# josegarciav/PINNs-RL-PDE

Hardware: AMD Instinct MI355X
Metric: collocation-points/sec (residual+grad) + final residual L2, Burgers 1D (higher is better)
Workload: dtype f32

## Files before the change

### pinns-rl-pde_amd/csrc/jet_kernel_u16.h

```cpp
#pragma once
#include "jet_kernel_wide.h"

namespace pinn {

#define U16_BARRIER(idx)     \
  do {                       \
    PINN_STAMP(idx);         \
    __syncthreads();         \
    PINN_STAMP(ST_BARRIER);  \
  } while (0)

constexpr int kU = 16;
constexpr int kUP = 132;
constexpr int kUThreads = 512;
constexpr int kUWaves = 8;
constexpr int kUH = 128;
constexpr int kUImgS = kU * kUP;

__device__ __forceinline__ f32x4 mfma16(float a, float b, f32x4 c) {
  return __builtin_amdgcn_mfma_f32_16x16x4f32(a, b, c, 0, 0, 0);
}

__device__ __forceinline__ int u16_opaque(int v) {
  asm volatile("" : "+v"(v));
// ... 87 lines not shown
__device__ __forceinline__ void u16_gemm_n(f32x4 (&acc)[K], const float* W, int ld, unsigned off, f32x4 w0, f32x4 w1, const float* xl) {
  f32x4 wq[3];
  wq[0] = w0;
  wq[1] = w1;
  f32x4 bc[K], bn[K];
#pragma unroll
  for (int s = 0; s < K; ++s) bc[s] = *reinterpret_cast<const f32x4*>(xl + s * kUImgS);
#pragma unroll
  for (int b = 0; b < NB; ++b) {
    if (b + 2 < NB) wq[(b + 2) % 3] = u16_wload<COLS>(W, ld, off, b + 2);
    if (b + 1 < NB) {
#pragma unroll
      for (int s = 0; s < K; ++s) bn[s] = *reinterpret_cast<const f32x4*>(xl + s * kUImgS + 16 * (b + 1));
    }
    __builtin_amdgcn_sched_barrier(0);
#pragma unroll
    for (int m = 0; m < 4; ++m)
#pragma unroll
      for (int s = 0; s < K; ++s) acc[s] = mfma16(wq[b % 3][m], bc[s][m], acc[s]);
    __builtin_amdgcn_sched_barrier(0);
    if (b + 1 < NB) {
#pragma unroll
      for (int s = 0; s < K; ++s) bc[s] = bn[s];
    }
  }
}

template <int K, bool COLS>
__device__ __forceinline__ void u16_gemm(f32x4 (&acc)[K], const float* W, int ld, unsigned off, f32x4 w0, f32x4 w1, int nb, const float* xl) {
  switch (nb) {
    case 8: u16_gemm_n<K, 8, COLS>(acc, W, ld, off, w0, w1, xl); return;
    case 4: u16_gemm_n<K, 4, COLS>(acc, W, ld, off, w0, w1, xl); return;
    default: break;
  }
#pragma unroll 1
  for (int b = 0; b < nb; ++b) {
    const f32x4 w = b == 0 ? w0 : b == 1 ? w1 : u16_wload<COLS>(W, ld, off, b);
#pragma unroll
    for (int m = 0; m < 4; ++m)
#pragma unroll
      for (int s = 0; s < K; ++s) acc[s] = mfma16(w[m], xl[s * kUImgS + 16 * b + m], acc[s]);
  }
}

template <int K, int NA, int OFF, int NPT>
__device__ __forceinline__ void u16_outer_n(f32x4 (&pt)[NPT], const float* zl, const float* al) {
  float zc, zn, ac[NA], an[NA];
  zc = zl[0];
#pragma unroll
  for (int t = 0; t < NA; ++t) ac[t] = al[16 * t];
#pragma unroll
  for (int st = 0; st < 4 * K; ++st) {
    if (st + 1 < 4 * K) {
      const int s = (st + 1) >> 2, m = (st + 1) & 3;
      zn = zl[s * kUImgS + m * kUP];
#pragma unroll
      for (int t = 0; t < NA; ++t) an[t] = al[s * kUImgS + m * kUP + 16 * t];
    }
    __builtin_amdgcn_sched_barrier(0);
#pragma unroll
    for (int t = 0; t < NA; ++t) pt[OFF + t] = mfma16(zc, ac[t], pt[OFF + t]);
    __builtin_amdgcn_sched_barrier(0);
    if (st + 1 < 4 * K) {
      zc = zn;
#pragma unroll
      for (int t = 0; t < NA; ++t) ac[t] = an[t];
    }
  }
}

template <int K, int OFF, int NMAX, int NPT>
__device__ __forceinline__ void u16_outer(f32x4 (&pt)[NPT], int na, const float* zl, const float* al) {
  if constexpr (NMAX >= 8) {
    if (na * 2 == NMAX) { u16_outer_n<K, NMAX / 2, OFF, NPT>(pt, zl, al); return; }
  }
  u16_outer_n<K, NMAX, OFF, NPT>(pt, zl, al);
}

#ifndef PINN_U16_PACK
#define PINN_U16_PACK 1
#endif
constexpr int kUPackMax = 3;

template <int NB, bool COLS>
__device__ __forceinline__ void u16p_gemm_n(f32x4 (&acc)[kUPackMax], int G, const float* W, int ld, unsigned off, f32x4 w0, f32x4 w1, const float* xl) {
  f32x4 wq[3];
  wq[0] = w0;
  wq[1] = w1;
  f32x4 bc[kUPackMax], bn[kUPackMax];
#pragma unroll
  for (int j = 0; j < kUPackMax; ++j) {
    bc[j] = f32x4{0.0f, 0.0f, 0.0f, 0.0f};
    bn[j] = bc[j];
    if (j < G) bc[j] = *reinterpret_cast<const f32x4*>(xl + 4 * j * kUP);
  }
#pragma unroll
  for (int b = 0; b < NB; ++b) {
    if (b + 2 < NB) wq[(b + 2) % 3] = u16_wload<COLS>(W, ld, off, b + 2);
    if (b + 1 < NB) {
#pragma unroll
      for (int j = 0; j < kUPackMax; ++j)
        if (j < G) bn[j] = *reinterpret_cast<const f32x4*>(xl + 4 * j * kUP + 16 * (b + 1));
    }
#pragma unroll
    for (int j = 0; j < kUPackMax; ++j) {
      if (j < G) {
#pragma unroll
        for (int m = 0; m < 4; ++m) acc[j] = mfma16(wq[b % 3][m], bc[j][m], acc[j]);
      }
    }
    if (b + 1 < NB) {
#pragma unroll
      for (int j = 0; j < kUPackMax; ++j) bc[j] = bn[j];
    }
  }
}

template <bool COLS>
__device__ __forceinline__ void u16p_gemm(f32x4 (&acc)[kUPackMax], int G, const float* W, int ld, unsigned off, f32x4 w0, f32x4 w1, int nb, const float* xl) {
  switch (nb) {
    case 8: u16p_gemm_n<8, COLS>(acc, G, W, ld, off, w0, w1, xl); return;
    case 4: u16p_gemm_n<4, COLS>(acc, G, W, ld, off, w0, w1, xl); return;
    default: break;
  }
#pragma unroll 1
  for (int b = 0; b < nb; ++b) {
    const f32x4 w = b == 0 ? w0 : b == 1 ? w1 : u16_wload<COLS>(W, ld, off, b);
#pragma unroll
    for (int j = 0; j < kUPackMax; ++j) {
      if (j < G) {
#pragma unroll
        for (int m = 0; m < 4; ++m) acc[j] = mfma16(w[m], xl[4 * j * kUP + 16 * b + m], acc[j]);
      }
    }
  }
}

template <int K, int NA, int OFF, int NPT>
__device__ __forceinline__ void u16p_outer_n(f32x4 (&pt)[NPT], int G, const float* zl, const float* al) {
#pragma unroll
  for (int j = 0; j < kUPackMax; ++j) {
    if (j < G) {
      float zc, zn = 0.0f, ac[NA], an[NA];
      zc = zl[4 * j * kUP];
#pragma unroll
      for (int t = 0; t < NA; ++t) {
        ac[t] = al[4 * j * kUP + 16 * t];
        an[t] = 0.0f;
      }
#pragma unroll
      for (int s = 0; s < K; ++s) {
        if (s + 1 < K) {
          zn = zl[(s + 1) * kUImgS + 4 * j * kUP];
#pragma unroll
          for (int t = 0; t < NA; ++t) an[t] = al[(s + 1) * kUImgS + 4 * j * kUP + 16 * t];
        }
        __builtin_amdgcn_sched_barrier(0);
#pragma unroll
        for (int t = 0; t < NA; ++t) pt[OFF + t] = mfma16(zc, ac[t], pt[OFF + t]);
        __builtin_amdgcn_sched_barrier(0);
        if (s + 1 < K) {
          zc = zn;
#pragma unroll
          for (int t = 0; t < NA; ++t) ac[t] = an[t];
        }
      }
// ... 9 lines not shown
  u16p_outer_n<K, NMAX, OFF, NPT>(pt, G, zl, al);
}

__device__ __forceinline__ void u16_wave_sync() {
  __builtin_amdgcn_fence(__ATOMIC_RELEASE, "wavefront");
  __builtin_amdgcn_wave_barrier();
  __builtin_amdgcn_fence(__ATOMIC_ACQUIRE, "wavefront");
}

template <int ACT, int NT, int NX, bool MRG = false>
__device__ __forceinline__ void u16_ew_forward(f32x4 (&v)[1 + NT + NX], float w, f32x4 (&rec)[1 + NT + NX], float cc = 0.0f) {
  constexpr int K = 1 + NT + NX;
#pragma unroll
  for (int r = 0; r < 4; ++r) {
    float z[K], y[K];
#pragma unroll
    for (int s = 0; s < K; ++s) z[s] = v[s][r];
    if constexpr (MRG) act_fwd_merged<ACT>(w, cc, z, y);
    else act_fwd<ACT, NT, NX>(w, z, y);
    rec[0][r] = ActTape<ACT>::value_is_output ? y[0] : z[0];
#pragma unroll
    for (int s = 1; s < K; ++s) rec[s][r] = z[s];
#pragma unroll
    for (int s = 0; s < K; ++s) v[s][r] = y[s];
  }
}

template <int K>
__device__ __forceinline__ void u16_put(float* il, const f32x4 (&v)[K]) {
#pragma unroll
  for (int s = 0; s < K; ++s) *reinterpret_cast<f32x4*>(il + s * kUImgS) = v[s];
}
template <int K>
__device__ __forceinline__ void u16_get(const float* il, f32x4 (&v)[K]) {
#pragma unroll
  for (int s = 0; s < K; ++s) v[s] = *reinterpret_cast<const f32x4*>(il + s * kUImgS);
}

template <int ACT, int NT, int NX, bool MRG = false>
__device__ __forceinline__ float u16_ew_backward(f32x4 (&ab)[1 + NT + NX], float w, const f32x4 (&rec)[1 + NT + NX], float cc = 0.0f) {
  constexpr int K = 1 + NT + NX;
  float part = 0.0f;
#pragma unroll
  for (int r = 0; r < 4; ++r) {
    float z[K], abv[K], zb[K];
#pragma unroll
    for (int s = 0; s < K; ++s) {
      z[s] = rec[s][r];
      abv[s] = ab[s][r];
    }
    if constexpr (MRG) part += act_bwd_tape_merged<ACT>(w, cc, z, abv, zb);
    else act_bwd_tape<ACT, NT, NX>(w, z, abv, zb);
#pragma unroll
    for (int s = 0; s < K; ++s) ab[s][r] = zb[s];
  }
  return part;
}

template <int ACT, int NT, int NX, bool MRG>
__device__ __forceinline__ void u16_act_replay(float w, float cc, const float* z, float* y) {
  if constexpr (MRG) act_fwd_tape_merged<ACT>(w, cc, z, y);
  else act_fwd_tape<ACT, NT, NX>(w, z, y);
}

__device__ __forceinline__ f32x4 row16_sum4(f32x4 v) {
#pragma unroll
  for (int r = 0; r < 4; ++r) v[r] = row16_sum(v[r]);
  return v;
}

template <int ACT, int NT, int NX, bool BWD, int NA0, bool COEF = false, bool MRG = false>
__global__ __launch_bounds__(kUThreads, 1) void jet_kernel_u16(const KernelArgs a) {
  static_assert(!MRG || (NT == 1 && NX == 1), "the merged set is laid out as the (1,1) set");
  constexpr int K = 1 + NT + NX;
  constexpr int NKT = kUH / 16;
  constexpr int NPT = NA0 + (kPersist - 1) * NKT;
  static_assert(kPersist == 3, "the layer -> tile-offset table below is written for three persistent layers");
  constexpr int img = K * kUImgS;
  extern __shared__ __attribute__((aligned(16))) float smem[];
  const NetDev& net = a.net;
  float* X = smem;
  float* A2 = X + img;
  float* REC = A2 + img;
  float* UP = REC + 2 * img;
  float* xin2 = UP + kUWaves * K * kU;
  float* wb = xin2 + 2 * kMaxDin * kU;
  float* ep = wb + (1 + kPersist) * kUH;
  float* pl = ep + (kMaxDin + 1) * kUH;
  float* pdwl = pl + (kPersist + kMaxDin + 1) * kUH;
  float* psl = pdwl + 4 * kUThreads;
  float* xint = psl + 2 * kU;
  [[maybe_unused]] float* pcl = xint + kMaxDin * kU;
  auto mcoef = [&]() -> float {
    if constexpr (MRG) return -X[kUH + 2];
    else return 0.0f;
  };
  auto cadd = [&](float part, bool own) {
    if constexpr (MRG && COEF) {
      if (own) pcl[u16_opaque(threadIdx.x)] += part;
    }
  };

  PINN_STAMP_DECL
  const int tid = threadIdx.x;
  const int wv = __builtin_amdgcn_readfirstlane(tid >> 6);
  const int lane = tid & 63;
  const int g = lane >> 4, c = lane & 15;
  const int din = net.din;
  const int nl = net.n_layers;
#if PINN_U16_PACK
  const long long NL = a.u16_loop_points;
#else
  const long long NL = a.N;
#endif
  const long long nunits = (NL + kU - 1) / kU;
  const int frow = 16 * wv + 4 * g;
  const int ioff = c * kUP + frow;

  for (int k = tid; k < kUH; k += kUThreads) {
    wb[k] = k < net.h_last ? net.w_out[k] : 0.0f;
    for (int l = 0; l < nl; ++l) wb[(1 + l) * kUH + k] = k < net.layer[l].out_dim ? net.layer[l].b[k] : 0.0f;
  }
  stage_enc_params<kUH>(net, ep, tid);
#pragma unroll
  for (int i = 0; i < kPersist + kMaxDin + 1; ++i)
    if (tid < kUH) pl[i * kUH + tid] = 0.0f;
  const float b_out0 = net.b_out[0];
  static_assert(!COEF || BWD, "coefficient cotangents belong to the reverse launch");
  if constexpr (COEF) {
    if (tid < kU) {
      X[tid * kUP + kUH] = 0.0f;
      X[tid * kUP + kUH + 1] = 0.0f;
    }
  }
  if (tid < 4) {
    const float cv = tid == 0 ? a.pde.c0 : tid == 1 ? a.pde.c1 : tid == 2 ? a.pde.c2 : a.pde.c3;
    X[tid * kUP + kUH + 2] = COEF ? a.pde.coef_dev[tid] : cv;
  }

  f32x4 pt[NPT];
#pragma unroll
  for (int t = 0; t < NPT; ++t) pt[t] = f32x4{0.0f, 0.0f, 0.0f, 0.0f};
  if constexpr (BWD) *reinterpret_cast<f32x4*>(pdwl + 4 * tid) = f32x4{0.0f, 0.0f, 0.0f, 0.0f};
  if (tid < 2 * kU) psl[tid] = 0.0f;
  if constexpr (MRG && COEF) pcl[tid] = 0.0f;

  float xr[kMaxDin] = {0.0f, 0.0f, 0.0f, 0.0f};
  auto fetch_coords = [&](long long u) {
    if (tid < kU) {
      const long long p = u * kU + tid;
      const bool ok = u < nunits && p < NL;
#pragma unroll
      for (int cc = 0; cc < kMaxDin; ++cc) {
        if (cc < din - 1) xr[cc] = ok ? a.x[p * (din - 1) + cc] : 0.0f;
        if (cc == din - 1) xr[cc] = ok ? a.t[p] : 0.0f;
      }
    }
  };
  auto fetch_coords_at = [&](long long p0, int npts) {
    if (tid < kU) {
      const long long p = p0 + tid;
      const bool ok = tid < npts && p < a.N;
#pragma unroll
      for (int cc = 0; cc < kMaxDin; ++cc) {
        if (cc < din - 1) xr[cc] = ok ? a.x[p * (din - 1) + cc] : 0.0f;
        if (cc == din - 1) xr[cc] = ok ? a.t[p] : 0.0f;
      }
    }
  };
  auto put_coords = [&](float* dst) {
    if (tid < kU) {
#pragma unroll
      for (int cc = 0; cc < kMaxDin; ++cc) dst[cc * kU + tid] = xr[cc];
    }
  };
#if PINN_U16_PACK
  if (a.u16_tail_groups > 0) {
    fetch_coords_at(a.u16_loop_points + 4LL * a.u16_tail_groups * blockIdx.x, 4 * a.u16_tail_groups);
    put_coords(xint);
  }
#endif
  fetch_coords(blockIdx.x);
  put_coords(xin2);
  int xpar = 0;

  for (long long u = blockIdx.x; u < nunits; u += gridDim.x) {
    const long long p0 = u * kU;
    U16_BARRIER(ST_BWD_FLUSH);
    const float* xin = xin2 + xpar * (kMaxDin * kU);
    float* xin_next = xin2 + (xpar ^ 1) * (kMaxDin * kU);
    xpar ^= 1;
    fetch_coords(u + gridDim.x);
    f32x4 w0, w1;
    {
      const LayerDev L0 = uniform_layer(net.layer[0]);
      const unsigned off = u16_rows_off(16 * wv < L0.out_dim ? 16 * wv : 0, L0.ld, c, g);
      w0 = u16_wload<false>(L0.W, L0.ld, off, 0);
      w1 = u16_wload<false>(L0.W, L0.ld, off, L0.in_dim > 16 ? 1 : 0);
    }
    PINN_STAMP(ST_STAGE);
    float* src = (nl & 1) ? X : A2;
    float* dst = (nl & 1) ? A2 : X;
    u16_encode<ACT, NT, NX, MRG>(net, ep, xin, src, u16_opaque(tid), mcoef());
    U16_BARRIER(ST_ENCODE);

    f32x4 acc[K];
    for (int l = 0; l < nl; ++l) {
      const LayerDev Ly = uniform_layer(net.layer[l]);
      const bool on = 16 * wv < Ly.out_dim;
      const bool last = l + 1 == nl;
#pragma unroll
      for (int s = 0; s < K; ++s) acc[s] = f32x4{0.0f, 0.0f, 0.0f, 0.0f};
      if (on) {
        u16_gemm<K, false>(acc, Ly.W, Ly.ld, u16_rows_off(16 * wv, Ly.ld, c, g), w0, w1, Ly.in_dim >> 4, src + c * kUP + 4 * g);
        acc[0] += *reinterpret_cast<const f32x4*>(wb + (1 + l) * kUH + frow);
      }
      if (l == 0) put_coords(xin_next);
      PINN_STAMP(ST_FWD_GEMM);
      if (!last) {
        {
          const LayerDev Ln = uniform_layer(net.layer[l + 1]);
          const unsigned off = u16_rows_off(16 * wv < Ln.out_dim ? 16 * wv : 0, Ln.ld, c, g);
          w0 = u16_wload<false>(Ln.W, Ln.ld, off, 0);
          w1 = u16_wload<false>(Ln.W, Ln.ld, off, Ln.in_dim > 16 ? 1 : 0);
        }
        if (on) {
          f32x4 rec[K];
          u16_ew_forward<ACT, NT, NX, MRG>(acc, Ly.act_param, rec, mcoef());
          if constexpr (BWD) u16_put<K>(REC + l * img + ioff, rec);
        }
        if (on) u16_put<K>(dst + ioff, acc);
        U16_BARRIER(ST_FWD_EW);
        float* const t = src;
        src = dst;
        dst = t;
      } else if (on) {
        f32x4 rec[K];
        u16_ew_forward<ACT, NT, NX, MRG>(acc, Ly.act_param, rec, mcoef());
        if constexpr (BWD) u16_put<K>(A2 + ioff, rec);
      }
    }
    PINN_STAMP(ST_FWD_EW);

    {
      const f32x4 w4 = *reinterpret_cast<const f32x4*>(wb + frow);
      float po[K];
#pragma unroll
      for (int s = 0; s < K; ++s) {
        po[s] = fmaf(w4[0], acc[s][0], fmaf(w4[1], acc[s][1], fmaf(w4[2], acc[s][2], w4[3] * acc[s][3])));
        po[s] += __shfl_xor(po[s], 16);
        po[s] += __shfl_xor(po[s], 32);
      }
      if (g == 0) {
#pragma unroll
        for (int s = 0; s < K; ++s) UP[(wv * K + s) * kU + c] = po[s];
      }
    }
    U16_BARRIER(ST_OUT);

    float ub[K];
    {
      const long long p = p0 + c;
      const bool ok = p < NL;
      const bool writer = tid < kU;
      float j[K];
#pragma unroll
      for (int s = 0; s < K; ++s) {
        float v = s == 0 ? b_out0 : 0.0f;
#pragma unroll
        for (int w = 0; w < kUWaves; ++w) v += UP[(w * K + s) * kU + c];
        j[s] = v;
      }
      if (a.mode == MODE_JETS) {
#pragma unroll
        for (int s = 0; s < K; ++s) {
          if (writer && ok && a.jets_out[s]) a.jets_out[s][p] = j[s];
          ub[s] = (BWD && ok && a.jets_bar[s]) ? a.jets_bar[s][p] : 0.0f;
        }
      } else {
        float d[K];
        PdeDev pde = a.pde;
        pde.c0 = X[0 * kUP + kUH + 2];
        pde.c1 = X[1 * kUP + kUH + 2];
        pde.c2 = X[2 * kUP + kUH + 2];
        pde.c3 = X[3 * kUP + kUH + 2];
        float r;
        if constexpr (MRG) r = pde_residual_merged(j, d);
        else r = pde_residual<NT, NX>(pde, j, xin[c], d);
        float dl;
        float lt = loss_term(pde, r, &dl);
        if (!ok) {
          lt = 0.0f;
          dl = 0.0f;
        }
        if (writer && ok && a.residual_out) a.residual_out[p] = r;
        if (writer) psl[c] += lt;
        const float rb = !BWD ? 0.0f : a.res_bar ? (ok ? a.res_bar[p] : 0.0f) : a.grad_scale * dl;
#pragma unroll
        for (int s = 0; s < K; ++s) ub[s] = rb * d[s];
        if constexpr (COEF && !MRG) {
          float dc0, dc1;
          pde_coef_grads<NT, NX>(pde, j, xin[c], dc0, dc1);
          if (writer) {
            X[c * kUP + kUH] += rb * dc0;
            X[c * kUP + kUH + 1] += rb * dc1;
          }
        }
      }
    }

    PINN_STAMP(ST_EPI);
    if constexpr (!BWD) continue;
    if (tid < kU) psl[kU + c] += ub[0];
    f32x4 ab[K];
    {
      const LayerDev Lz = uniform_layer(net.layer[nl - 1]);
      const f32x4 w4 = *reinterpret_cast<const f32x4*>(wb + frow);
#pragma unroll
      for (int s = 0; s < K; ++s) ab[s] = w4 * ub[s];
      if (16 * wv < Lz.out_dim) {
        f32x4 rec[K];
        u16_get<K>(A2 + ioff, rec);
        float* const pdwp = pdwl + 4 * u16_opaque(tid);
        f32x4 pdw = *reinterpret_cast<const f32x4*>(pdwp);
#pragma unroll
        for (int r = 0; r < 4; ++r) {
          float z[K], y[K];
#pragma unroll
          for (int s = 0; s < K; ++s) z[s] = rec[s][r];
          u16_act_replay<ACT, NT, NX, MRG>(Lz.act_param, mcoef(), z, y);
          float gg = 0.0f;
#pragma unroll
          for (int s = 0; s < K; ++s) gg = fmaf(ub[s], y[s], gg);
          pdw[r] += gg;
        }
        *reinterpret_cast<f32x4*>(pdwp) = pdw;
        cadd(u16_ew_backward<ACT, NT, NX, MRG>(ab, Lz.act_param, rec, mcoef()), true);
      }
    }
    PINN_STAMP(ST_B0);

    for (int l = nl - 1; l >= 0; --l) {
      const LayerDev Ly = uniform_layer(net.layer[l]);
      const bool on = 16 * wv < Ly.out_dim;
      const bool need_abar = l > 0 || net.enc == ENC_LINEAR;
      const bool kon = 16 * wv < Ly.in_dim;
      if (l + 1 < nl || nl == 1) U16_BARRIER(ST_BWD_EW);
      if (on) u16_put<K>(X + ioff, ab);
      float pw = 0.0f;
      if (l > 0) {
        const LayerDev P = uniform_layer(net.layer[l - 1]);
        pw = P.act_param;
        if (kon) {
          f32x4 rec[K], y[K];
          u16_get<K>(REC + (l - 1) * img + ioff, rec);
#pragma unroll
          for (int r = 0; r < 4; ++r) {
            float z[K], yy[K];
#pragma unroll
            for (int s = 0; s < K; ++s) z[s] = rec[s][r];
            u16_act_replay<ACT, NT, NX, MRG>(pw, mcoef(), z, yy);
#pragma unroll
            for (int s = 0; s < K; ++s) y[s][r] = yy[s];
          }
          u16_put<K>(A2 + ioff, y);
        }
      } else {
        u16_encode<ACT, NT, NX, MRG>(net, ep, xin, A2, u16_opaque(tid), mcoef());
      }
      const unsigned coff = u16_cols_off(kon ? 16 * wv : 0, Ly.ld, c, g);
      if (need_abar) {
        w0 = u16_wload<true>(Ly.W, Ly.ld, coff, 0);
        w1 = u16_wload<true>(Ly.W, Ly.ld, coff, 1);
      }
      U16_BARRIER(ST_BWD_PUT);
      if (Ly.db && tid < Ly.out_dim) {
        float gsum = 0.0f;
#pragma unroll
        for (int n = 0; n < kU; ++n) gsum += X[n * kUP + tid];
        pl[l * kUH + tid] += gsum;
      }
      PINN_STAMP(ST_BWD_DB);
      const bool dw_first = wv >= 4;
#pragma unroll
      for (int half = 0; half < 2; ++half) {
        if ((half == 0) == dw_first && on && Ly.dW) {
          const float* zl = X + 4 * g * kUP + 16 * wv + c;
          const float* al = A2 + 4 * g * kUP + c;
          const int na = Ly.in_dim >> 4;
          if (l == 0) u16_outer<K, 0, NA0, NPT>(pt, na, zl, al);
          else if (l == 1) u16_outer<K, NA0, NKT, NPT>(pt, na, zl, al);
          else u16_outer<K, NA0 + NKT, NKT, NPT>(pt, na, zl, al);
        }
        if ((half == 0) == dw_first) PINN_STAMP(ST_BWD_STREAM);
        if (half == 1) break;
        if (need_abar) {
#pragma unroll
          for (int s = 0; s < K; ++s) ab[s] = f32x4{0.0f, 0.0f, 0.0f, 0.0f};
          if (kon) u16_gemm<K, true>(ab, Ly.W, Ly.ld, coff, w0, w1, Ly.out_dim >> 4, X + c * kUP + 4 * g);
        }
        PINN_STAMP(ST_BWD_DX);
        if (l > 0 && kon) {
          f32x4 rec[K];
          u16_get<K>(REC + (l - 1) * img + ioff, rec);
          cadd(u16_ew_backward<ACT, NT, NX, MRG>(ab, pw, rec, mcoef()), true);
        }
        PINN_STAMP(ST_BWD_EW);
      }
      if constexpr (MRG && COEF) {
        if (l == 0 && net.enc == ENC_FOURIER && kon) {
          f32x4 aw[1] = {f32x4{0.0f, 0.0f, 0.0f, 0.0f}};
          {
            const float* xl = X + kUImgS + c * kUP + 4 * g;
            const int nb = Ly.out_dim >> 4;
#pragma unroll 1
            for (int b = 0; b < nb; ++b) {
              const f32x4 w = u16_wload<true>(Ly.W, Ly.ld, coff, b);
              const f32x4 xv = *reinterpret_cast<const f32x4*>(xl + 16 * b);
#pragma unroll
              for (int m = 0; m < 4; ++m) aw[0] = mfma16(w[m], xv[m], aw[0]);
            }
          }
          const int M = net.enc_out >> 1;
          const f32x4 val = *reinterpret_cast<const f32x4*>(A2 + ioff);
          float part = 0.0f;
#pragma unroll
          for (int r = 0; r < 4; ++r) {
            const int jf = frow + r;
            part = fmaf(aw[0][r], fourier_coef_partial_merged(ep[jf < M ? jf : jf - M], val[r]), part);
          }
          cadd(part, true);
        }
      }
    }

    if (net.enc == ENC_LINEAR && (net.d_encW || (MRG && COEF))) {
      const int H = net.enc_out;
      const bool enc_sums = !(MRG && COEF) || net.d_encW != nullptr;
      U16_BARRIER(ST_ENC_BWD);
      if (16 * wv < H) {
#pragma unroll
        for (int r = 0; r < 4; ++r) {
          float z[K], abv[K], zb[K];
          u16_enc_preact<NT, NX>(ep, din, xin, frow + r, c, z);
#pragma unroll
          for (int s = 0; s < K; ++s) abv[s] = ab[s][r];
          if constexpr (MRG) cadd(act_bwd_merged<ACT>(net.enc_param, mcoef(), z, abv, zb), true);
          else act_bwd<ACT, NT, NX>(net.enc_param, z, abv, zb);
#pragma unroll
          for (int s = 0; s < K; ++s) ab[s][r] = zb[s];
        }
        if (enc_sums) u16_put<K>(X + ioff, ab);
      }
      U16_BARRIER(ST_ENC_BWD);
      const int te = u16_opaque(tid);
      if (enc_sums && te < H) {
        float gb = 0.0f, gt = 0.0f, gx = 0.0f;
        float gw[kMaxDin] = {0.0f, 0.0f, 0.0f, 0.0f};
#pragma unroll 4
        for (int n = 0; n < kU; ++n) {
          const float vv = X[n * kUP + te];
          gb += vv;
#pragma unroll
          for (int cc = 0; cc < kMaxDin; ++cc)
            if (cc < din) gw[cc] = fmaf(vv, xin[cc * kU + n], gw[cc]);
          if constexpr (NT >= 1) gt += X[1 * kUImgS + n * kUP + te];
          if constexpr (NX >= 1) gx += X[(1 + NT) * kUImgS + n * kUP + te];
        }
#pragma unroll
        for (int cc = 0; cc < kMaxDin; ++cc) pl[(kPersist + cc) * kUH + te] += gw[cc] + (cc == din - 1 ? gt : 0.0f) + (cc == 0 ? gx : 0.0f);
        pl[(kPersist + kMaxDin) * kUH + te] += gb;
      }
      PINN_STAMP(ST_ENC_BWD);
    }
  }

#if PINN_U16_PACK
  if (a.u16_tail_groups > 0) {
    const int G = a.u16_tail_groups;
    const int tp = u16_opaque(tid);
    const int gp = (tp & 63) >> 4, cp = tp & 15;
    const int sp = cp >> 2, qp = cp & 3;
    const int frowp = 16 * wv + 4 * gp;
    const int boff = (sp < K ? sp : 0) * kUImgS + qp * kUP + 4 * gp;
    const int woff = sp * kUImgS + qp * kUP + frowp;
    const int eoff = qp * kUP + frowp;
    const bool wcol = sp < K;
    const bool writer = tp < 4;
    const long long tail_p0 = a.u16_loop_points + 4LL * G * blockIdx.x;
    auto acc_put = [&](float* im, const f32x4 (&pa)[kUPackMax]) {
#pragma unroll
      for (int j = 0; j < kUPackMax; ++j)
        if (j < G && wcol) *reinterpret_cast<f32x4*>(im + woff + 4 * j * kUP) = pa[j];
      u16_wave_sync();
    };

    U16_BARRIER(ST_BWD_FLUSH);
    const float* xin = xint;
    f32x4 w0, w1;
    {
      const LayerDev L0 = uniform_layer(net.layer[0]);
      const unsigned off = u16_rows_off(16 * wv < L0.out_dim ? 16 * wv : 0, L0.ld, cp, gp);
      w0 = u16_wload<false>(L0.W, L0.ld, off, 0);
      w1 = u16_wload<false>(L0.W, L0.ld, off, L0.in_dim > 16 ? 1 : 0);
    }
    PINN_STAMP(ST_STAGE);
    float* src = (nl & 1) ? X : A2;
// ... 246 lines not shown
        if (on && Ly.dW) {
          const float* zl = X + gp * kUP + 16 * wv + cp;
          const float* al = A2 + gp * kUP + cp;
          const int na = Ly.in_dim >> 4;
          if (l == 0) u16p_outer<K, 0, NA0, NPT>(pt, G, na, zl, al);
          else if (l == 1) u16p_outer<K, NA0, NKT, NPT>(pt, G, na, zl, al);
          else u16p_outer<K, NA0 + NKT, NKT, NPT>(pt, G, na, zl, al);
        }
        PINN_STAMP(ST_BWD_STREAM);
        if constexpr (MRG && COEF) {
          if (l == 0 && net.enc == ENC_FOURIER && kon) {
            f32x4 pa[kUPackMax];
#pragma unroll
            for (int j = 0; j < kUPackMax; ++j) pa[j] = f32x4{0.0f, 0.0f, 0.0f, 0.0f};
            u16p_gemm<true>(pa, G, Ly.W, Ly.ld, coff, u16_wload<true>(Ly.W, Ly.ld, coff, 0), u16_wload<true>(Ly.W, Ly.ld, coff, 1),
                            Ly.out_dim >> 4, X + boff);
            const int M = net.enc_out >> 1;
            float part = 0.0f;
#pragma unroll
            for (int j = 0; j < kUPackMax; ++j) {
              if (j < G) {
                const f32x4 val = *reinterpret_cast<const f32x4*>(A2 + eoff + 4 * j * kUP);
#pragma unroll
                for (int r = 0; r < 4; ++r) {
                  const int jf = frowp + r;
                  part = fmaf(pa[j][r], fourier_coef_partial_merged(ep[jf < M ? jf : jf - M], val[r]), part);
                }
              }
            }
            cadd(part, sp == 1);
          }
        }
      }

      if (net.enc == ENC_LINEAR && (net.d_encW || (MRG && COEF))) {
        const int H = net.enc_out;
        const bool enc_sums = !(MRG && COEF) || net.d_encW != nullptr;
        U16_BARRIER(ST_ENC_BWD);
        if (16 * wv < H) {
#pragma unroll
          for (int j = 0; j < kUPackMax; ++j) {
            if (j < G) {
              f32x4 ab[K];
              u16_get<K>(park + eoff + 4 * j * kUP, ab);
#pragma unroll
              for (int r = 0; r < 4; ++r) {
                float z[K], abv[K], zb[K];
                u16_enc_preact<NT, NX>(ep, din, xin, frowp + r, 4 * j + qp, z);
#pragma unroll
                for (int s = 0; s < K; ++s) abv[s] = ab[s][r];
                if constexpr (MRG) cadd(act_bwd_merged<ACT>(net.enc_param, mcoef(), z, abv, zb), sp == 0);
                else act_bwd<ACT, NT, NX>(net.enc_param, z, abv, zb);
#pragma unroll
                for (int s = 0; s < K; ++s) ab[s][r] = zb[s];
              }
              if (enc_sums) u16_put<K>(X + eoff + 4 * j * kUP, ab);
            }
          }
        }
        U16_BARRIER(ST_ENC_BWD);
        if (enc_sums && tp < H) {
          float gb = 0.0f, gt = 0.0f, gx = 0.0f;
          float gw[kMaxDin] = {0.0f, 0.0f, 0.0f, 0.0f};
          for (int n = 0; n < 4 * G; ++n) {
            const float vv = X[n * kUP + tp];
            gb += vv;
#pragma unroll
            for (int cc = 0; cc < kMaxDin; ++cc)
              if (cc < din) gw[cc] = fmaf(vv, xin[cc * kU + n], gw[cc]);
            if constexpr (NT >= 1) gt += X[1 * kUImgS + n * kUP + tp];
            if constexpr (NX >= 1) gx += X[(1 + NT) * kUImgS + n * kUP + tp];
          }
#pragma unroll
          for (int cc = 0; cc < kMaxDin; ++cc) pl[(kPersist + cc) * kUH + tp] += gw[cc] + (cc == din - 1 ? gt : 0.0f) + (cc == 0 ? gx : 0.0f);
          pl[(kPersist + kMaxDin) * kUH + tp] += gb;
        }
        PINN_STAMP(ST_ENC_BWD);
      }
    }
    __syncthreads();
  }
#endif

  const int tf = u16_opaque(tid);
  const int cf = tf & 15, frowf = 16 * wv + 4 * ((tf & 63) >> 4);
  const long long doff = det_row_offset(a);
  if (a.mode == MODE_PDE && a.loss_sum && wv == 0) {
    float sacc = tf < kU ? psl[tf] : 0.0f;
#pragma unroll
    for (int o = 8; o > 0; o >>= 1) sacc += __shfl_xor(sacc, o);
    if (tf == 0) grad_put(a.loss_sum, sacc, doff, a.flush_store != 0);
  }
#ifdef PINN_STAMPS
  auto write_stamps = [&]() {
    if (a.stamps && (tf & 63) == 0) {
      st_acc[ST_TOTAL] = pinn_now() - st_begin;
      for (int i = 0; i < kNumStamps; ++i) a.stamps[((long long)blockIdx.x * kUWaves + wv) * kNumStamps + i] = st_acc[i];
    }
  };
  if constexpr (!BWD) write_stamps();
#endif
  if constexpr (!BWD) return;
  if constexpr (COEF && MRG) {
    float sc = pcl[tf];
#pragma unroll
    for (int o = 32; o > 0; o >>= 1) sc += __shfl_xor(sc, o);
    if ((tf & 63) == 0) UP[wv] = sc;
    __syncthreads();
    if (a.mode == MODE_PDE && a.pde.dcoef && tf == 0) {
      float st = 0.0f;
#pragma unroll
      for (int w = 0; w < kUWaves; ++w) st += UP[w];
      a.pde.dcoef[doff] = -st;
      a.pde.dcoef[doff + 1] = 0.0f;
    }
  } else if constexpr (COEF) {
    if (a.mode == MODE_PDE && a.pde.dcoef && wv == 0) {
      float s0 = tf < kU ? X[tf * kUP + kUH] : 0.0f, s1 = tf < kU ? X[tf * kUP + kUH + 1] : 0.0f;
#pragma unroll
      for (int o = 8; o > 0; o >>= 1) {
        s0 += __shfl_xor(s0, o);
        s1 += __shfl_xor(s1, o);
      }
      if (tf == 0) {
        a.pde.dcoef[doff] = s0;
        a.pde.dcoef[doff + 1] = s1;
      }
    }
  }
  if (net.db_out && wv == 0) {
    float gsum = tf < kU ? psl[kU + tf] : 0.0f;
#pragma unroll
    for (int o = 8; o > 0; o >>= 1) gsum += __shfl_xor(gsum, o);
    if (tf == 0) net.db_out[doff] = gsum;
  }
  if (net.enc == ENC_LINEAR && net.d_encW && tf < net.enc_out) {
#pragma unroll
    for (int cc = 0; cc < kMaxDin; ++cc)
      if (cc < din) net.d_encW[doff + tf * din + cc] = pl[(kPersist + cc) * kUH + tf];
    if (net.d_encb) net.d_encb[doff + tf] = pl[(kPersist + kMaxDin) * kUH + tf];
  }
  const f32x4 pdw = row16_sum4(*reinterpret_cast<const f32x4*>(pdwl + 4 * tf));
  if (net.dw_out && cf == 0 && frowf < net.h_last) *reinterpret_cast<f32x4*>(net.dw_out + doff + frowf) = pdw;
#pragma unroll
  for (int p = 0; p < kPersist; ++p) {
    if (p < nl) {
      const LayerDev Lp = uniform_layer(net.layer[p]);
      if (Lp.db && tf < Lp.out_dim) Lp.db[doff + tf] = pl[p * kUH + tf];
      if (16 * wv >= Lp.out_dim) continue;
      if (Lp.dW) {
        const int na = Lp.in_dim >> 4;
        const int off = p == 0 ? 0 : p == 1 ? NA0 : NA0 + NKT;
        float* base = Lp.dW + doff + (long long)frowf * Lp.ld + cf;
#pragma unroll
        for (int t = 0; t < NPT; ++t) {
          if (t >= off && t - off < na && (p != 0 || t < NA0) && (p != 1 || t < NA0 + NKT)) {
#pragma unroll
            for (int r = 0; r < 4; ++r) base[(long long)r * Lp.ld + 16 * (t - off)] = pt[t][r];
          }
        }
      }
    }
  }
#ifdef PINN_STAMPS
  PINN_STAMP(ST_BWD_FLUSH);
  write_stamps();
#endif
}

struct U16Plan {
  long long rounds;
  long long first_tail;
  int groups;
};
inline U16Plan jet_u16_tail_plan(long long N, int grid, bool packed) {
  U16Plan p;
  const long long per_round = (long long)kU * grid;
  p.rounds = N / per_round;
  p.first_tail = p.rounds * per_round;
  const long long M = N - p.first_tail;
  p.groups = (int)((M + 4LL * grid - 1) / (4LL * grid));
  if (!packed && p.groups > 0) p.groups = 4;
  return p;
}
inline void jet_u16_set_plan(KernelArgs& a, int grid, bool packed) {
  const U16Plan p = jet_u16_tail_plan(a.N, grid, packed);
  const bool pack = p.groups >= 1 && p.groups <= kUPackMax;
  a.u16_loop_points = pack ? p.first_tail : a.N;
  a.u16_tail_groups = pack ? p.groups : 0;
}

inline size_t jet_u16_lds_bytes(int K) {
  return sizeof(float) * ((size_t)4 * K * kUImgS + kUWaves * K * kU + 2 * kMaxDin * kU + (1 + kPersist) * kUH +
                          (kMaxDin + 1) * kUH + (kPersist + kMaxDin + 1) * kUH + 4 * kUThreads + 2 * kU + kMaxDin * kU);
}
inline size_t jet_u16m_lds_bytes(bool coef) { return jet_u16_lds_bytes(3) + (coef ? sizeof(float) * kUThreads : 0); }


inline bool jet_u16_fits(const NetDev& n, int K) {
  if (K > 4 || n.n_layers < 1 || n.n_layers > kPersist || jet_wide_hmax(n.hmax) != 128) return false;
  if (n.layer[0].in_dim > 64) return false;
  for (int l = 0; l < n.n_layers; ++l)
    if (n.layer[l].in_dim % 16 || n.layer[l].out_dim % 16 || n.layer[l].in_dim > kUH || n.layer[l].out_dim > kUH) return false;
  return jet_u16_lds_bytes(K) <= 160 * 1024;
}

template <int ACT, int NT, int NX>
hipError_t launch_jet_u16_act(const KernelArgs& a, bool bwd, int grid, hipStream_t stream) {
  constexpr int K = 1 + NT + NX;
  auto kern = bwd ? jet_kernel_u16<ACT, NT, NX, true, 4> : jet_kernel_u16<ACT, NT, NX, false, 4>;
  hipError_t e = allow_full_lds(reinterpret_cast<const void*>(kern));
  if (e != hipSuccess) return e;
  hipLaunchKernelGGL(kern, dim3(grid), dim3(kUThreads), jet_u16_lds_bytes(K), stream, a);
  return hipGetLastError();
}

template <int ACT, int NT, int NX>
hipError_t launch_jet_u16_coef(const KernelArgs& a, int grid, hipStream_t stream) {
  constexpr int K = 1 + NT + NX;
  auto kern = jet_kernel_u16<ACT, NT, NX, true, 4, true>;
  hipError_t e = allow_full_lds(reinterpret_cast<const void*>(kern));
  if (e != hipSuccess) return e;
  hipLaunchKernelGGL(kern, dim3(grid), dim3(kUThreads), jet_u16_lds_bytes(K), stream, a);
  return hipGetLastError();
}

template <int ACT>
hipError_t launch_jet_u16m_act(const KernelArgs& a, bool bwd, int grid, hipStream_t stream) {
  auto kern = bwd ? jet_kernel_u16<ACT, 1, 1, true, 4, false, true> : jet_kernel_u16<ACT, 1, 1, false, 4, false, true>;
  hipError_t e = allow_full_lds(reinterpret_cast<const void*>(kern));
  if (e != hipSuccess) return e;
  hipLaunchKernelGGL(kern, dim3(grid), dim3(kUThreads), jet_u16m_lds_bytes(false), stream, a);
  return hipGetLastError();
}
template <int ACT>
hipError_t launch_jet_u16m_coef(const KernelArgs& a, int grid, hipStream_t stream) {
  auto kern = jet_kernel_u16<ACT, 1, 1, true, 4, true, true>;
  hipError_t e = allow_full_lds(reinterpret_cast<const void*>(kern));
  if (e != hipSuccess) return e;
  hipLaunchKernelGGL(kern, dim3(grid), dim3(kUThreads), jet_u16m_lds_bytes(true), stream, a);
  return hipGetLastError();
}

}
```

Before: 130.5 million.

## Double-buffer merged backward layer images and accumulate bias grads in registers

In the merged (MRG) reverse kernel, the backward layer loop now alternates between two LDS image sets (X/A2 and a new S/REC1 buffer). While the current layer's GEMM reads one set, the next layer's cotangent and replayed activations are written into the other. This removes one block barrier per layer. Bias gradients are also kept in per-thread register accumulators and reduced once at the end, replacing the per-layer LDS column sum. The cost is extra LDS (three more image slices) and more registers.

```diff
diff --git a/pinns-rl-pde_amd/csrc/jet_kernel_u16.h b/pinns-rl-pde_amd/csrc/jet_kernel_u16.h
--- a/pinns-rl-pde_amd/csrc/jet_kernel_u16.h
+++ b/pinns-rl-pde_amd/csrc/jet_kernel_u16.h
@@ -193,6 +193,13 @@
 #endif
 constexpr int kUPackMax = 3;
 
+#ifndef PINN_U16M_SWEEP
+#define PINN_U16M_SWEEP 1
+#endif
+#ifndef PINN_U16M_DBREG
+#define PINN_U16M_DBREG 1
+#endif
+
 template <int NB, bool COLS>
 __device__ __forceinline__ void u16p_gemm_n(f32x4 (&acc)[kUPackMax], int G, const float* W, int ld, unsigned off, f32x4 w0, f32x4 w1, const float* xl) {
   f32x4 wq[3];
@@ -377,6 +384,10 @@
   float* psl = pdwl + 4 * kUThreads;
   float* xint = psl + 2 * kU;
   [[maybe_unused]] float* pcl = xint + kMaxDin * kU;
+  constexpr bool SWP = MRG && BWD && PINN_U16M_SWEEP;
+  constexpr bool DBR = MRG && BWD && PINN_U16M_DBREG;
+  [[maybe_unused]] float* S = pcl + (COEF ? kUThreads : 0);
+  [[maybe_unused]] float* REC1 = REC + img;
   auto mcoef = [&]() -> float {
     if constexpr (MRG) return -X[kUH + 2];
     else return 0.0f;
@@ -427,6 +438,18 @@
   f32x4 pt[NPT];
 #pragma unroll
   for (int t = 0; t < NPT; ++t) pt[t] = f32x4{0.0f, 0.0f, 0.0f, 0.0f};
+  [[maybe_unused]] f32x4 dbacc[kPersist];
+  if constexpr (DBR) {
+#pragma unroll
+    for (int p = 0; p < kPersist; ++p) dbacc[p] = f32x4{0.0f, 0.0f, 0.0f, 0.0f};
+  }
+  [[maybe_unused]] auto db_add = [&](int l, const f32x4& zb) {
+    if constexpr (DBR) {
+#pragma unroll
+      for (int p = 0; p < kPersist; ++p)
+        if (p == l) dbacc[p] += zb;
+    }
+  };
   if constexpr (BWD) *reinterpret_cast<f32x4*>(pdwl + 4 * tid) = f32x4{0.0f, 0.0f, 0.0f, 0.0f};
   if (tid < 2 * kU) psl[tid] = 0.0f;
   if constexpr (MRG && COEF) pcl[tid] = 0.0f;
@@ -622,6 +645,7 @@
         }
         *reinterpret_cast<f32x4*>(pdwp) = pdw;
         cadd(u16_ew_backward<ACT, NT, NX, MRG>(ab, Lz.act_param, rec, mcoef()), true);
+        db_add(nl - 1, ab[0]);
       }
     }
     PINN_STAMP(ST_B0);
@@ -631,28 +655,71 @@
       const bool on = 16 * wv < Ly.out_dim;
       const bool need_abar = l > 0 || net.enc == ENC_LINEAR;
       const bool kon = 16 * wv < Ly.in_dim;
-      if (l + 1 < nl || nl == 1) U16_BARRIER(ST_BWD_EW);
-      if (on) u16_put<K>(X + ioff, ab);
+      float* Zi = X;
+      float* Ai = A2;
       float pw = 0.0f;
-      if (l > 0) {
-        const LayerDev P = uniform_layer(net.layer[l - 1]);
-        pw = P.act_param;
-        if (kon) {
-          f32x4 rec[K], y[K];
-          u16_get<K>(REC + (l - 1) * img + ioff, rec);
-#pragma unroll
-          for (int r = 0; r < 4; ++r) {
-            float z[K], yy[K];
-#pragma unroll
-            for (int s = 0; s < K; ++s) z[s] = rec[s][r];
-            u16_act_replay<ACT, NT, NX, MRG>(pw, mcoef(), z, yy);
-#pragma unroll
-            for (int s = 0; s < K; ++s) y[s][r] = yy[s];
-          }
-          u16_put<K>(A2 + ioff, y);
+      [[maybe_unused]] float* Zn = X;
+      [[maybe_unused]] float* An = A2;
+      [[maybe_unused]] auto put_replay = [&](int lz, bool zon, bool aon, float* Zd, float* Ad) {
+        if (zon) u16_put<K>(Zd + ioff, ab);
+        if (lz > 0) {
+          const float pwz = uniform_layer(net.layer[lz - 1]).act_param;
+          if (aon) {
+            f32x4 rec[K], y[K];
+            u16_get<K>(REC + (lz - 1) * img + ioff, rec);
+#pragma unroll
+            for (int r = 0; r < 4; ++r) {
+              float z[K], yy[K];
+#pragma unroll
+              for (int s = 0; s < K; ++s) z[s] = rec[s][r];
+              u16_act_replay<ACT, NT, NX, MRG>(pwz, mcoef(), z, yy);
+#pragma unroll
+              for (int s = 0; s < K; ++s) y[s][r] = yy[s];
+            }
+            u16_put<K>(Ad + ioff, y);
+          }
+        } else {
+          u16_encode<ACT, NT, NX, MRG>(net, ep, xin, Ad, u16_opaque(tid), mcoef());
+        }
+      };
+      if constexpr (!MRG) {
+        if (l + 1 < nl || nl == 1) U16_BARRIER(ST_BWD_EW);
+        if (on) u16_put<K>(X + ioff, ab);
+        if (l > 0) {
+          const LayerDev P = uniform_layer(net.layer[l - 1]);
+          pw = P.act_param;
+          if (kon) {
+            f32x4 rec[K], y[K];
+            u16_get<K>(REC + (l - 1) * img + ioff, rec);
+#pragma unroll
+            for (int r = 0; r < 4; ++r) {
+              float z[K], yy[K];
+#pragma unroll
+              for (int s = 0; s < K; ++s) z[s] = rec[s][r];
+              u16_act_replay<ACT, NT, NX, MRG>(pw, mcoef(), z, yy);
+#pragma unroll
+              for (int s = 0; s < K; ++s) y[s][r] = yy[s];
+            }
+            u16_put<K>(A2 + ioff, y);
+          }
+        } else {
+          u16_encode<ACT, NT, NX, MRG>(net, ep, xin, A2, u16_opaque(tid), mcoef());
         }
       } else {
-        u16_encode<ACT, NT, NX, MRG>(net, ep, xin, A2, u16_opaque(tid), mcoef());
+        bool open = true;
+        if constexpr (SWP) {
+          const bool odd = (nl - 1 - l) & 1;
+          Zi = odd ? S : X;
+          Ai = odd ? REC1 : A2;
+          Zn = odd ? X : S;
+          An = odd ? A2 : REC1;
+          open = l + 1 == nl;
+        }
+        if (l > 0) pw = uniform_layer(net.layer[l - 1]).act_param;
+        if (open) {
+          if (l + 1 < nl || nl == 1) U16_BARRIER(ST_BWD_EW);
+          put_replay(l, on, kon, Zi, Ai);
+        }
       }
       const unsigned coff = u16_cols_off(kon ? 16 * wv : 0, Ly.ld, c, g);
       if (need_abar) {
@@ -660,19 +727,21 @@
         w1 = u16_wload<true>(Ly.W, Ly.ld, coff, 1);
       }
       U16_BARRIER(ST_BWD_PUT);
-      if (Ly.db && tid < Ly.out_dim) {
-        float gsum = 0.0f;
-#pragma unroll
-        for (int n = 0; n < kU; ++n) gsum += X[n * kUP + tid];
-        pl[l * kUH + tid] += gsum;
+      if constexpr (!DBR) {
+        if (Ly.db && tid < Ly.out_dim) {
+          float gsum = 0.0f;
+#pragma unroll
+          for (int n = 0; n < kU; ++n) gsum += Zi[n * kUP + tid];
+          pl[l * kUH + tid] += gsum;
+        }
       }
       PINN_STAMP(ST_BWD_DB);
       const bool dw_first = wv >= 4;
 #pragma unroll
       for (int half = 0; half < 2; ++half) {
         if ((half == 0) == dw_first && on && Ly.dW) {
-          const float* zl = X + 4 * g * kUP + 16 * wv + c;
-          const float* al = A2 + 4 * g * kUP + c;
+          const float* zl = Zi + 4 * g * kUP + 16 * wv + c;
+          const float* al = Ai + 4 * g * kUP + c;
           const int na = Ly.in_dim >> 4;
           if (l == 0) u16_outer<K, 0, NA0, NPT>(pt, na, zl, al);
           else if (l == 1) u16_outer<K, NA0, NKT, NPT>(pt, na, zl, al);
@@ -683,21 +752,28 @@
         if (need_abar) {
 #pragma unroll
           for (int s = 0; s < K; ++s) ab[s] = f32x4{0.0f, 0.0f, 0.0f, 0.0f};
-          if (kon) u16_gemm<K, true>(ab, Ly.W, Ly.ld, coff, w0, w1, Ly.out_dim >> 4, X + c * kUP + 4 * g);
+          if (kon) u16_gemm<K, true>(ab, Ly.W, Ly.ld, coff, w0, w1, Ly.out_dim >> 4, Zi + c * kUP + 4 * g);
         }
         PINN_STAMP(ST_BWD_DX);
         if (l > 0 && kon) {
           f32x4 rec[K];
           u16_get<K>(REC + (l - 1) * img + ioff, rec);
           cadd(u16_ew_backward<ACT, NT, NX, MRG>(ab, pw, rec, mcoef()), true);
+          db_add(l - 1, ab[0]);
         }
         PINN_STAMP(ST_BWD_EW);
+        if constexpr (SWP) {
+          if (l > 0) {
+            put_replay(l - 1, kon, 16 * wv < uniform_layer(net.layer[l - 1]).in_dim, Zn, An);
+            PINN_STAMP(ST_BWD_PUT);
+          }
+        }
       }
       if constexpr (MRG && COEF) {
         if (l == 0 && net.enc == ENC_FOURIER && kon) {
           f32x4 aw[1] = {f32x4{0.0f, 0.0f, 0.0f, 0.0f}};
           {
-            const float* xl = X + kUImgS + c * kUP + 4 * g;
+            const float* xl = Zi + kUImgS + c * kUP + 4 * g;
             const int nb = Ly.out_dim >> 4;
 #pragma unroll 1
             for (int b = 0; b < nb; ++b) {
@@ -708,7 +784,7 @@
             }
           }
           const int M = net.enc_out >> 1;
-          const f32x4 val = *reinterpret_cast<const f32x4*>(A2 + ioff);
+          const f32x4 val = *reinterpret_cast<const f32x4*>(Ai + ioff);
           float part = 0.0f;
 #pragma unroll
           for (int r = 0; r < 4; ++r) {
@@ -1121,6 +1197,22 @@
   }
 #endif
 
+  if constexpr (DBR) {
+    __syncthreads();
+#pragma unroll
+    for (int p = 0; p < kPersist; ++p) {
+      if (p < nl) {
+        const LayerDev Lp = uniform_layer(net.layer[p]);
+        if (Lp.db && 16 * wv < Lp.out_dim) {
+          const f32x4 sd = row16_sum4(dbacc[p]);
+          float* const pr = pl + p * kUH + 16 * wv + 4 * ((u16_opaque(tid) & 63) >> 4);
+          if ((u16_opaque(tid) & 15) == 0) *reinterpret_cast<f32x4*>(pr) = *reinterpret_cast<const f32x4*>(pr) + sd;
+        }
+      }
+    }
+    __syncthreads();
+  }
+
   const int tf = u16_opaque(tid);
   const int cf = tf & 15, frowf = 16 * wv + 4 * ((tf & 63) >> 4);
   const long long doff = det_row_offset(a);
@@ -1233,7 +1325,12 @@
   return sizeof(float) * ((size_t)4 * K * kUImgS + kUWaves * K * kU + 2 * kMaxDin * kU + (1 + kPersist) * kUH +
                           (kMaxDin + 1) * kUH + (kPersist + kMaxDin + 1) * kUH + 4 * kUThreads + 2 * kU + kMaxDin * kU);
 }
-inline size_t jet_u16m_lds_bytes(bool coef) { return jet_u16_lds_bytes(3) + (coef ? sizeof(float) * kUThreads : 0); }
+inline constexpr size_t jet_u16m_lds_bytes(bool coef, bool bwd) {
+  return sizeof(float) * ((size_t)4 * 3 * kUImgS + kUWaves * 3 * kU + 2 * kMaxDin * kU + (1 + kPersist) * kUH + (kMaxDin + 1) * kUH +
+                          (kPersist + kMaxDin + 1) * kUH + 4 * kUThreads + 2 * kU + kMaxDin * kU + (coef ? kUThreads : 0) +
+                          (bwd && PINN_U16M_SWEEP ? 3 * kUImgS : 0));
+}
+static_assert(jet_u16m_lds_bytes(true, true) <= 160 * 1024, "the merged COEF reverse launch must fit the 160 KB of LDS");
 
 
 inline bool jet_u16_fits(const NetDev& n, int K) {
@@ -1269,7 +1366,7 @@
   auto kern = bwd ? jet_kernel_u16<ACT, 1, 1, true, 4, false, true> : jet_kernel_u16<ACT, 1, 1, false, 4, false, true>;
   hipError_t e = allow_full_lds(reinterpret_cast<const void*>(kern));
   if (e != hipSuccess) return e;
-  hipLaunchKernelGGL(kern, dim3(grid), dim3(kUThreads), jet_u16m_lds_bytes(false), stream, a);
+  hipLaunchKernelGGL(kern, dim3(grid), dim3(kUThreads), jet_u16m_lds_bytes(false, bwd), stream, a);
   return hipGetLastError();
 }
 template <int ACT>
@@ -1277,7 +1374,7 @@
   auto kern = jet_kernel_u16<ACT, 1, 1, true, 4, true, true>;
   hipError_t e = allow_full_lds(reinterpret_cast<const void*>(kern));
   if (e != hipSuccess) return e;
-  hipLaunchKernelGGL(kern, dim3(grid), dim3(kUThreads), jet_u16m_lds_bytes(true), stream, a);
+  hipLaunchKernelGGL(kern, dim3(grid), dim3(kUThreads), jet_u16m_lds_bytes(true, true), stream, a);
   return hipGetLastError();
 }
 
```

New measurement: 130.3 million. Within noise of the previous version (-0.2%).

## Keep backward adjoints in LDS for merged kernel to skip activation replay

Applied to the files above, without the earlier changes.

For the merged (MRG) backward kernel, a fifth LDS image is added so the last layer's record and each layer's adjoint are kept in place instead of being recomputed. This removes the per-layer activation replay and some barriers in the backward pass, reads z/a operands directly from the stored REC/S images, and re-encodes inputs only when needed. The cost is larger LDS allocation per block and more complex buffer aliasing (src/dst parity forced), which risks correctness if the buffer reuse is wrong.

```diff
diff --git a/pinns-rl-pde_amd/csrc/jet_kernel_u16.h b/pinns-rl-pde_amd/csrc/jet_kernel_u16.h
--- a/pinns-rl-pde_amd/csrc/jet_kernel_u16.h
+++ b/pinns-rl-pde_amd/csrc/jet_kernel_u16.h
@@ -368,7 +368,9 @@
   float* X = smem;
   float* A2 = X + img;
   float* REC = A2 + img;
-  float* UP = REC + 2 * img;
+  constexpr bool KEEP = MRG && BWD;
+  [[maybe_unused]] float* S = REC + 2 * img;
+  float* UP = REC + (KEEP ? 3 : 2) * img;
   float* xin2 = UP + kUWaves * K * kU;
   float* wb = xin2 + 2 * kMaxDin * kU;
   float* ep = wb + (1 + kPersist) * kUH;
@@ -485,8 +487,8 @@
       w1 = u16_wload<false>(L0.W, L0.ld, off, L0.in_dim > 16 ? 1 : 0);
     }
     PINN_STAMP(ST_STAGE);
-    float* src = (nl & 1) ? X : A2;
-    float* dst = (nl & 1) ? A2 : X;
+    float* src = (MRG || (nl & 1)) ? X : A2;
+    float* dst = (MRG || (nl & 1)) ? A2 : X;
     u16_encode<ACT, NT, NX, MRG>(net, ep, xin, src, u16_opaque(tid), mcoef());
     U16_BARRIER(ST_ENCODE);
 
@@ -523,7 +525,7 @@
       } else if (on) {
         f32x4 rec[K];
         u16_ew_forward<ACT, NT, NX, MRG>(acc, Ly.act_param, rec, mcoef());
-        if constexpr (BWD) u16_put<K>(A2 + ioff, rec);
+        if constexpr (BWD) u16_put<K>((KEEP ? S : A2) + ioff, rec);
       }
     }
     PINN_STAMP(ST_FWD_EW);
@@ -606,7 +608,7 @@
       for (int s = 0; s < K; ++s) ab[s] = w4 * ub[s];
       if (16 * wv < Lz.out_dim) {
         f32x4 rec[K];
-        u16_get<K>(A2 + ioff, rec);
+        u16_get<K>((KEEP ? S : A2) + ioff, rec);
         float* const pdwp = pdwl + 4 * u16_opaque(tid);
         f32x4 pdw = *reinterpret_cast<const f32x4*>(pdwp);
 #pragma unroll
@@ -614,7 +616,12 @@
           float z[K], y[K];
 #pragma unroll
           for (int s = 0; s < K; ++s) z[s] = rec[s][r];
-          u16_act_replay<ACT, NT, NX, MRG>(Lz.act_param, mcoef(), z, y);
+          if constexpr (KEEP) {
+#pragma unroll
+            for (int s = 0; s < K; ++s) y[s] = acc[s][r];
+          } else {
+            u16_act_replay<ACT, NT, NX, MRG>(Lz.act_param, mcoef(), z, y);
+          }
           float gg = 0.0f;
 #pragma unroll
           for (int s = 0; s < K; ++s) gg = fmaf(ub[s], y[s], gg);
@@ -622,6 +629,7 @@
         }
         *reinterpret_cast<f32x4*>(pdwp) = pdw;
         cadd(u16_ew_backward<ACT, NT, NX, MRG>(ab, Lz.act_param, rec, mcoef()), true);
+        if constexpr (KEEP) u16_put<K>(S + ioff, ab);
       }
     }
     PINN_STAMP(ST_B0);
@@ -631,10 +639,16 @@
       const bool on = 16 * wv < Ly.out_dim;
       const bool need_abar = l > 0 || net.enc == ENC_LINEAR;
       const bool kon = 16 * wv < Ly.in_dim;
-      if (l + 1 < nl || nl == 1) U16_BARRIER(ST_BWD_EW);
-      if (on) u16_put<K>(X + ioff, ab);
+      if constexpr (!KEEP) {
+        if (l + 1 < nl || nl == 1) U16_BARRIER(ST_BWD_EW);
+        if (on) u16_put<K>(X + ioff, ab);
+      }
+      const float* const ZB = !KEEP ? X : l + 1 == nl ? S : REC + l * img;
+      const float* const AP = !KEEP || (l & 1) ? A2 : X;
       float pw = 0.0f;
-      if (l > 0) {
+      if constexpr (KEEP) {
+        if (l > 0) pw = uniform_layer(net.layer[l - 1]).act_param;
+      } else if (l > 0) {
         const LayerDev P = uniform_layer(net.layer[l - 1]);
         pw = P.act_param;
         if (kon) {
@@ -663,7 +677,7 @@
       if (Ly.db && tid < Ly.out_dim) {
         float gsum = 0.0f;
 #pragma unroll
-        for (int n = 0; n < kU; ++n) gsum += X[n * kUP + tid];
+        for (int n = 0; n < kU; ++n) gsum += ZB[n * kUP + tid];
         pl[l * kUH + tid] += gsum;
       }
       PINN_STAMP(ST_BWD_DB);
@@ -671,8 +685,8 @@
 #pragma unroll
       for (int half = 0; half < 2; ++half) {
         if ((half == 0) == dw_first && on && Ly.dW) {
-          const float* zl = X + 4 * g * kUP + 16 * wv + c;
-          const float* al = A2 + 4 * g * kUP + c;
+          const float* zl = ZB + 4 * g * kUP + 16 * wv + c;
+          const float* al = AP + 4 * g * kUP + c;
           const int na = Ly.in_dim >> 4;
           if (l == 0) u16_outer<K, 0, NA0, NPT>(pt, na, zl, al);
           else if (l == 1) u16_outer<K, NA0, NKT, NPT>(pt, na, zl, al);
@@ -683,21 +697,28 @@
         if (need_abar) {
 #pragma unroll
           for (int s = 0; s < K; ++s) ab[s] = f32x4{0.0f, 0.0f, 0.0f, 0.0f};
-          if (kon) u16_gemm<K, true>(ab, Ly.W, Ly.ld, coff, w0, w1, Ly.out_dim >> 4, X + c * kUP + 4 * g);
+          if (kon) u16_gemm<K, true>(ab, Ly.W, Ly.ld, coff, w0, w1, Ly.out_dim >> 4, ZB + c * kUP + 4 * g);
         }
         PINN_STAMP(ST_BWD_DX);
         if (l > 0 && kon) {
           f32x4 rec[K];
           u16_get<K>(REC + (l - 1) * img + ioff, rec);
           cadd(u16_ew_backward<ACT, NT, NX, MRG>(ab, pw, rec, mcoef()), true);
+          if constexpr (KEEP) u16_put<K>(REC + (l - 1) * img + ioff, ab);
         }
         PINN_STAMP(ST_BWD_EW);
+      }
+      if constexpr (KEEP) {
+        if (l == 1 && nl > 2) {
+          u16_encode<ACT, NT, NX, MRG>(net, ep, xin, X, u16_opaque(tid), mcoef());
+          PINN_STAMP(ST_ENCODE);
+        }
       }
       if constexpr (MRG && COEF) {
         if (l == 0 && net.enc == ENC_FOURIER && kon) {
           f32x4 aw[1] = {f32x4{0.0f, 0.0f, 0.0f, 0.0f}};
           {
-            const float* xl = X + kUImgS + c * kUP + 4 * g;
+            const float* xl = ZB + kUImgS + c * kUP + 4 * g;
             const int nb = Ly.out_dim >> 4;
 #pragma unroll 1
             for (int b = 0; b < nb; ++b) {
@@ -708,7 +729,7 @@
             }
           }
           const int M = net.enc_out >> 1;
-          const f32x4 val = *reinterpret_cast<const f32x4*>(A2 + ioff);
+          const f32x4 val = *reinterpret_cast<const f32x4*>(AP + ioff);
           float part = 0.0f;
 #pragma unroll
           for (int r = 0; r < 4; ++r) {
@@ -1233,7 +1254,14 @@
   return sizeof(float) * ((size_t)4 * K * kUImgS + kUWaves * K * kU + 2 * kMaxDin * kU + (1 + kPersist) * kUH +
                           (kMaxDin + 1) * kUH + (kPersist + kMaxDin + 1) * kUH + 4 * kUThreads + 2 * kU + kMaxDin * kU);
 }
-inline size_t jet_u16m_lds_bytes(bool coef) { return jet_u16_lds_bytes(3) + (coef ? sizeof(float) * kUThreads : 0); }
+constexpr size_t jet_u16m_lds_bytes(bool coef, bool bwd) {
+  return sizeof(float) * ((size_t)(bwd ? 5 : 4) * 3 * kUImgS + kUWaves * 3 * kU + 2 * kMaxDin * kU + (1 + kPersist) * kUH +
+                          (kMaxDin + 1) * kUH + (kPersist + kMaxDin + 1) * kUH + 4 * kUThreads + 2 * kU + kMaxDin * kU +
+                          (coef ? kUThreads : 0));
+}
+static_assert(jet_u16m_lds_bytes(true, true) <= 160 * 1024 && jet_u16m_lds_bytes(false, true) == 146048 &&
+                  jet_u16m_lds_bytes(false, false) == 120704,
+              "the merged units' five images and running sums fit the CU's LDS");
 
 
 inline bool jet_u16_fits(const NetDev& n, int K) {
@@ -1269,7 +1297,7 @@
   auto kern = bwd ? jet_kernel_u16<ACT, 1, 1, true, 4, false, true> : jet_kernel_u16<ACT, 1, 1, false, 4, false, true>;
   hipError_t e = allow_full_lds(reinterpret_cast<const void*>(kern));
   if (e != hipSuccess) return e;
-  hipLaunchKernelGGL(kern, dim3(grid), dim3(kUThreads), jet_u16m_lds_bytes(false), stream, a);
+  hipLaunchKernelGGL(kern, dim3(grid), dim3(kUThreads), jet_u16m_lds_bytes(false, bwd), stream, a);
   return hipGetLastError();
 }
 template <int ACT>
@@ -1277,7 +1305,7 @@
   auto kern = jet_kernel_u16<ACT, 1, 1, true, 4, true, true>;
   hipError_t e = allow_full_lds(reinterpret_cast<const void*>(kern));
   if (e != hipSuccess) return e;
-  hipLaunchKernelGGL(kern, dim3(grid), dim3(kUThreads), jet_u16m_lds_bytes(true), stream, a);
+  hipLaunchKernelGGL(kern, dim3(grid), dim3(kUThreads), jet_u16m_lds_bytes(true, true), stream, a);
   return hipGetLastError();
 }
 
```

After: 131.0 million before, 133.6 million after, median of 6. 1.02x the previous value.
